# JJKK1313/DiTreeOnlinePlanner

Measured on AMD Instinct MI355X. Metric: candidate tree-expansions/sec (carmaze, H=32), higher is better.
Workload: dtype f16x3; 1 GPU; cfgs/carmaze.yaml + fm_policy flow sampler (K=1), batch=1024 candidates per GPU, H=32 (4 chunks x 8 steps), boxes.csv 20x20, 1024-node tree snapshot, seeded random weights; batch_per_gpu=1024, global_batch=1024, edge_length=32, action_horizon=8, pred_horizon=64, flow_steps=1, tree_nodes=1024, parallelism=candidates sharded x1

## Files before the change

### ditreeonlineplanner_amd/csrc/denoise.h

```cpp
#pragma once
#include <hip/hip_runtime.h>
#include <stdint.h>

enum { MODE_BIAS = 0, MODE_GN_MISH = 1, MODE_GN_MISH_FILM = 2, MODE_GN_MISH_RES = 3 };

enum { ST_BF16 = 0, ST_F32 = 1, ST_F16 = 2 };
static inline int fmt_make(int st, bool split) { return st | (split ? 4 : 0); }
static inline __host__ __device__ int fmt_st(int f) { return f & 3; }
static inline __host__ __device__ bool fmt_split(int f) { return (f & 4) != 0; }
static inline int fmt_es(int f) { return fmt_st(f) == ST_F32 ? 4 : 2; }

struct ConvGemmParams {
  const void* A;
  int lda;
  int in_Lp;
  int in_stride;
  int in_off;
  int taps, Cin;
  const void* W;
  void* Out;
  int ldc;
  int out_Lp, out_stride, out_off;
  int out_coff;
  int L;
  int M, N;
  const float* bias;
  int mode;
  const float* gamma;
  const float* beta;
  int group_ch;
  float eps;
  const float* film;
  int film_ld, film_off;
  const void* Res;
  int ldres, res_Lp, res_off;
  int out_f32;
  int dbg;
  int c2d, c2_H, c2_W, c2_OW, c2_OHW, c2_stride, c2_pad;
  signed char c2_kh[12], c2_kw[12];
  const void* zero;
  long long a_plane, w_plane, out_plane, res_plane;
  float w_scale;
  int splitk;
  long long slab_stride;
  float* sk_ws;
  int* sk_cnt;
  int* sat;
};

void denoise_set_dry_run(bool on);
void launch_conv_gemm(const ConvGemmParams& p, int fmt, hipStream_t s);
bool conv2d_small_eligible(int fmt);
int conv_gemm_kind(const ConvGemmParams& p, int fmt);
bool conv_gemm_supported(const ConvGemmParams& p, int fmt);
void launch_prep_sample(const float* x, void* A0, int B, int P, int D, int fmt, long long plane, hipStream_t s, int* sat = nullptr);
void launch_time_embed(float t, const float* W1, const float* b1, const float* W2, const float* b2, float* out,
                       hipStream_t s);
void launch_prep_cond(const float* temb, const float* map_emb, int E, int E_ld, const float* cond, int G, void* out, int B,
                      int Kpad, int fmt, long long plane, hipStream_t s, int* sat = nullptr);
struct FlowStep {
  int mode;
  float dt;
  float sb, sa, c0, c1, sigma;
  const float* z;
  long long z_row;
  const int* z_idx;
  int z_row0;
};
void launch_final_proj_flow(const void* Y, int C, int Lp, long long plane, const float* W, const float* bias, int D, float* x,
                            FlowStep fs, const double* act_norm , double* actions, int B, int P, int fmt,
                            hipStream_t s);
struct TapList {
  int n;
  signed char kh[49], kw[49];
};
void launch_gn1d(void* x, int ld, int Lp, int row_off, int coff, int L, int C, const float* gamma, const float* beta, float eps,
                 int mode, const float* film, int film_ld, int film_off, const void* res, int ldres, int res_Lp, int res_off,
                 int B, int fmt, long long x_plane, long long res_plane, hipStream_t s, int* sat = nullptr);
void launch_encoder_stem(const float* lm, int n, const float* W, const float* gamma, const float* beta, void* out, int B, float eps,
                         int fmt, long long plane, hipStream_t s, int* sat = nullptr);
void launch_im2col2d(const void* in, bool src_f32, void* out, int B, int H, int W, int C, const TapList& taps, int stride,
                     int pad, int OH, int OW, int Kpad, int fmt, hipStream_t s);
// ... 9 lines not shown
```

### ditreeonlineplanner_amd/csrc/denoise_host.hip

```cpp
#include <algorithm>
#include <cmath>
#include <cstring>
#include <functional>
#include <map>
#include <sstream>
#include <thread>

#include "denoise.h"
#include "ditree_internal.h"

namespace {

struct HostParam {
  std::vector<int64_t> dims;
  const float* data = nullptr;
  int64_t n = 0;
};

struct Act {
  void* p = nullptr;
  int L = 0, C = 0;
  int ld = 0, coff = 0;
  bool padded = true;
  long long plane = 0;
// ... 41 lines not shown
  int bgran = 16;
  int ufmt = 0, efmt = 0;
  std::vector<void*> allocs;
  std::map<std::string, Act> named;
  std::map<std::string, Packed> dev_w;
  std::map<std::string, float*> dev_f;
  std::vector<std::function<void(int, int, hipStream_t)>> unet_ops;
  std::vector<std::function<void(int, int, int, hipStream_t)>> enc_ops;
  static constexpr int ENC_SUBS = 4;
  int sub_cap = 0;
  size_t col_region = 0, gout_region = 0;
  hipStream_t aux[ENC_SUBS] = {nullptr, nullptr, nullptr, nullptr};
  hipEvent_t ev_fork = nullptr, ev_join[ENC_SUBS] = {nullptr, nullptr, nullptr, nullptr};
  std::function<void(int, int, hipStream_t)> film_op;
  float* x_cur = nullptr;
  float* temb = nullptr;
  float temb_t = -1.0f;
  float* map_emb = nullptr;
  int E_ld = 400;
  float* film = nullptr;
  void* condA = nullptr;
  long long cond_plane = 0;
  int condK = 0, film_cols = 0;
  Act final_h;
  const float* lm_ptr = nullptr;
  void* zero_row = nullptr;
  static constexpr int SAT_SLOTS = 256;
  int* sat_flags = nullptr;
  int *sat_cond = nullptr, *sat_sample = nullptr;
  std::vector<std::string> sat_names;
  int* sat_slot(const std::string& layer, int fmt) {
    if (fmt_st(fmt) != ST_F16 || sat_flags == nullptr) return nullptr;
    for (size_t i = 0; i < sat_names.size(); ++i)
      if (sat_names[i] == layer) return sat_flags + i;
    if ((int)sat_names.size() >= SAT_SLOTS) return sat_flags + SAT_SLOTS - 1;
    sat_names.push_back(layer);
    return sat_flags + sat_names.size() - 1;
  }
  int last_splitk[4] = {1, 1, 1, 1};
  long long last_slab[4] = {0, 0, 0, 0};
  bool prof_on = false;
  int prof_mode = 0;
  std::vector<hipEvent_t> prof_ev;
  size_t prof_used = 0;
  double prof_ms_done[3] = {0, 0, 0};
  int64_t prof_launches_done[3] = {0, 0, 0};
// ... 98 lines not shown
    if (it == params.end()) throw std::runtime_error("missing parameter " + name);
    return it->second;
  }
  bool has(const std::string& name) const { return params.count(name) != 0; }

  void* dalloc(size_t bytes, bool zero = true) {
    void* p = nullptr;
    if (hipMalloc(&p, bytes ? bytes : 16) != hipSuccess) throw std::runtime_error("hipMalloc failed");
    if (zero && hipMemset(p, 0, bytes ? bytes : 16) != hipSuccess) throw std::runtime_error("hipMemset failed");
    allocs.push_back(p);
    return p;
  }
  void free_workspace() {
    for (void* p : allocs) hipFree(p);
    allocs.clear();
    sk_ws = nullptr;
    sk_cnt = nullptr;
    named.clear();
    dev_w.clear();
    dev_f.clear();
    enc_ops.clear();
    unet_ops.clear();
    film_op = nullptr;
    sat_flags = sat_cond = sat_sample = nullptr;
    sat_names.clear();
    prec = -1;
    Bmax = 0;
    Buser = 0;
    temb_t = -1.0f;
  }

  float* upload_f32(const std::string& key, const float* src, int64_t n) {
    auto it = dev_f.find(key);
    if (it != dev_f.end()) return it->second;
    float* d = (float*)dalloc((size_t)n * 4, false);
    if (hipMemcpy(d, src, (size_t)n * 4, hipMemcpyHostToDevice) != hipSuccess) throw std::runtime_error("memcpy");
    dev_f[key] = d;
    return d;
  }
  float* vec(const std::string& name) {
    const HostParam& hp = P_(name);
    return upload_f32(name, hp.data, hp.n);
  }

  template <class F>
  Packed pack(const std::string& key, int fmt, int N, int T, int Cin_pad, F get) {
// ... 218 lines not shown
    default: throw std::runtime_error("unknown precision");
  }
  sat_flags = (int*)dalloc(SAT_SLOTS * sizeof(int));
  sat_cond = sat_slot("cond_encoder input: Mish(time | map embedding | observation)", ufmt);
  sat_sample = sat_slot("sample (the noisy action sequence)", ufmt);
  const int C0 = dims[0], C1 = dims[1], C2 = dims[2];
  const int L0 = P, L1 = P / 2, L2 = P / 4;
  if (P % 16 != 0 || P < 16 || P > 256 || (256 % P) != 0) throw std::runtime_error("pred_horizon must be 16, 32, 64, 128 or 256");
  bgran = fmt_st(ufmt) != ST_F32 ? std::max(16, 1024 / P) : 16;
  Buser = Bmax_;
  Bmax = (Bmax_ + bgran - 1) / bgran * bgran;
  {
    const long long per_sample = std::max({(long long)(L2 + 2) * 2 * C2, (long long)(L1 + 2) * 2 * C1, (long long)(L0 + 2) * C0,
                                           (long long)L0 * 64}) * fmt_es(ufmt);
    long long cap = std::min<long long>(8192, 0x7f000000LL / per_sample);
    cap = cap / 256 * 256;
    if (cap < 256) throw std::runtime_error("denoiser too large for one 256-sample work unit");
    if (Bmax > cap) Bmax = (int)cap;
  }
  if (fmt_split(ufmt) && ((C0 | C1 | C2) & 255) != 0)
    throw std::runtime_error("the split precisions need down_dims that are multiples of 256 (halo / gemm16 tiles)");
  x_cur = (float*)dalloc((size_t)Bmax * P * D * 4);
  temb = (float*)dalloc(256 * 4);
  condK = (cond_dim + 63) / 64 * 64;
  const int Brows = (Bmax + 255) / 256 * 256;
  E_ld = fmt_split(efmt) ? (E + 255) / 256 * 256 : E;
  map_emb = (float*)dalloc((size_t)Brows * E_ld * 4);
  cond_plane = planes() == 2 ? (long long)Brows * condK * es() : 0;
  condA = dalloc((size_t)Brows * condK * es() * planes());

  std::vector<std::string> crbs = {"unet.down_modules.0.0", "unet.down_modules.0.1", "unet.down_modules.1.0",
                                   "unet.down_modules.1.1", "unet.down_modules.2.0", "unet.down_modules.2.1",
                                   "unet.mid_modules.0",    "unet.mid_modules.1",    "unet.up_modules.0.0",
                                   "unet.up_modules.0.1",   "unet.up_modules.1.0",   "unet.up_modules.1.1"};
  film_cols = 0;
  std::vector<int> film_offs;
  for (auto& c : crbs) {
    film_offs.push_back(film_cols);
    film_cols += (int)P_(c + ".cond_encoder.1.weight").dims[0];
  }
  film = (float*)dalloc((size_t)Brows * film_cols * 4);
  {
    std::vector<const float*> wsrc, bsrc;
    std::vector<int> rows;
    for (auto& c : crbs) {
      wsrc.push_back(P_(c + ".cond_encoder.1.weight").data);
      bsrc.push_back(P_(c + ".cond_encoder.1.bias").data);
      rows.push_back((int)P_(c + ".cond_encoder.1.weight").dims[0]);
    }
    std::vector<int> start(rows.size());
    for (size_t i = 0, a = 0; i < rows.size(); ++i) { start[i] = (int)a; a += rows[i]; }
    const int cd = cond_dim;
    const Packed wp = pack("film.all", ufmt, film_cols, 1, condK, [=](int n, int, int ci) {
      size_t i = std::upper_bound(start.begin(), start.end(), n) - start.begin() - 1;
      return ci < cd ? wsrc[i][(size_t)(n - start[i]) * cd + ci] : 0.0f;
    });
    std::vector<float> ball(film_cols);
    for (size_t i = 0; i < rows.size(); ++i) std::memcpy(ball.data() + start[i], bsrc[i], (size_t)rows[i] * 4);
    float* bd = upload_f32("film.bias", ball.data(), film_cols);
    ConvGemmParams p{};
    p.A = condA; p.lda = condK; p.in_Lp = 0; p.in_stride = 1; p.in_off = 0; p.taps = 1; p.Cin = condK;
    set_w(p, wp); p.a_plane = cond_plane;
    p.Out = film; p.ldc = film_cols; p.out_Lp = 0; p.out_stride = 1; p.out_off = 0;
    p.N = film_cols; p.bias = bd; p.mode = MODE_BIAS; p.out_f32 = 1;
    const int uf = ufmt;
    film_op = [this, p, uf](int, int Bp, hipStream_t s) mutable {
      const int Mr = fmt_st(uf) == ST_F32 ? Bp : (Bp + 255) / 256 * 256;
      p.M = Mr; p.L = Mr; p.in_Lp = Mr; p.out_Lp = Mr;
      run_gemm(p, uf, s);
    };
  }

  int fc = 0;
  Act a0;
  a0.L = L0; a0.C = 64; a0.ld = 64; a0.coff = 0; a0.padded = false; a0.fmt = ufmt;
  a0.plane = planes() == 2 ? (long long)Bmax * L0 * 64 * es() : 0;
  a0.p = dalloc((size_t)Bmax * L0 * 64 * es() * planes());
  named["a0"] = a0;
  {
    const std::string pre = "unet.down_modules.0.0";
    const HostParam& w = P_(pre + ".blocks.0.block.0.weight");
    const float* wd = w.data;
// ... 142 lines not shown
        float* goutr = gout + (size_t)reg * goutreg;
        ConvGemmParams p{};
        const int M = Bn * OH * OH;
        if (implicit) {
          p.A = (const char*)in + (size_t)b0 * H * H * Cin * E_; p.lda = Cin; p.taps = tl.n; p.Cin = Cin; p.a_plane = in_plane;
          p.c2d = 1; p.c2_H = H; p.c2_W = H; p.c2_OW = OH; p.c2_OHW = OH * OH; p.c2_stride = stride; p.c2_pad = pad;
          for (int t = 0; t < tl.n; ++t) { p.c2_kh[t] = tl.kh[t]; p.c2_kw[t] = tl.kw[t]; }
          p.zero = zr;
          const int nk_total = tl.n * (Cin / 64);
          const int tiles = ((1024 * OH * OH + 255) / 256) * ((Cout + 255) / 256);
          static int sk_target = -1, sk_cap = 8;
          if (sk_target < 0) {
            const char* e = getenv("DITREE_SPLITK_TARGET");
            sk_target = (e && atoi(e) > 0) ? atoi(e) : 256;
            const char* c = getenv("DITREE_SPLITK_CAP");
            if (c && atoi(c) > 0) sk_cap = atoi(c);
          }
          int sk = std::max(1, std::min(std::min(sk_cap, nk_total / 2), std::max(1, sk_target / tiles)));
          while (sk > 1 && (size_t)sk * OH * OH * Cout > gout_per_sample) --sk;
          if (sk > 1) {
            const int per = (nk_total + sk - 1) / sk;
            sk = (nk_total + per - 1) / per;
          }
          static int use_split = -1;
          if (use_split < 0) { const char* e = getenv("DITREE_SPLITK"); use_split = (e && !atoi(e)) ? 0 : 1; }
          if (conv2d_small_eligible(pr)) {
            static int small_target = -1;
            if (small_target < 0) { const char* e = getenv("DITREE_C2D_TARGET"); small_target = (e && atoi(e) > 0) ? atoi(e) : 768; }
            const int tiles64 = ((1024 * OH * OH + 63) / 64) * (Cout / 64);
            sk = std::max(1, std::min(std::min(8, nk_total / 2), small_target / tiles64));
            while (sk > 1 && (size_t)sk * OH * OH * Cout > gout_per_sample) --sk;
            if (sk > 1) {
              const int per = (nk_total + sk - 1) / sk;
              sk = (nk_total + per - 1) / per;
            }
          }
          if (!use_split) sk = 1;
          p.splitk = sk;
          p.slab_stride = (long long)M * Cout;
          last_splitk[reg] = sk;
          last_slab[reg] = p.slab_stride;
        } else {
          last_splitk[reg] = 1;
          last_slab[reg] = 0;
        }
        if (!implicit) {
          note_other();
          if (in == nullptr)
            launch_im2col2d(*lm_slot + (size_t)b0 * H * H, true, colr, Bn, H, H, 1, tl, stride, pad, OH, OH, Kpad, pr, s);
          else
            launch_im2col2d((const char*)in + (size_t)b0 * H * H * Cin * E_, false, colr, Bn, H, H, Cin, tl, stride, pad,
// ... 296 lines not shown
        HIP_TRY(ctx, hipEventCreateWithFlags(&st->ev_join[i], hipEventDisableTiming));
      }
      HIP_TRY(ctx, hipEventCreateWithFlags(&st->ev_fork, hipEventDisableTiming));
    }
    if (nsub > 1) HIP_TRY(ctx, hipEventRecord(st->ev_fork, s));
    for (int i = 0; i < nsub; ++i) {
      const int b0 = i * per, bn = std::min(per, B - b0);
      if (bn <= 0) break;
      hipStream_t si = (i == 0) ? s : st->aux[i];
      if (i > 0) HIP_TRY(ctx, hipStreamWaitEvent(si, st->ev_fork, 0));
      for (auto& op : st->enc_ops) op(b0, bn, i, si);
      if (i > 0) {
        HIP_TRY(ctx, hipEventRecord(st->ev_join[i], si));
        HIP_TRY(ctx, hipStreamWaitEvent(s, st->ev_join[i], 0));
      }
    }
  }
  for (int k = 0; k < K; ++k) {
    const float t = t0[k] * t_scale;
    if (t != st->temb_t) {
      launch_time_embed(t, st->dev_f["unet.diffusion_step_encoder.1.weight"], st->dev_f["unet.diffusion_step_encoder.1.bias"],
                        st->dev_f["unet.diffusion_step_encoder.3.weight"], st->dev_f["unet.diffusion_step_encoder.3.bias"],
                        st->temb, s);
      st->temb_t = K == 1 ? t : -1.0f;
    }
    st->note_other();
    launch_prep_cond(st->temb, st->map_emb, st->E, st->E_ld, cond, st->G, st->condA, B, st->condK, uf, st->cond_plane, s,
                     st->sat_cond);
    st->film_op(B, Bp, s);
    st->note_other();
    launch_prep_sample(st->x_cur, st->named["a0"].p, Bp, st->P, st->D, uf, st->named["a0"].plane, s,
                       st->sat_sample);
    for (auto& op : st->unet_ops) op(B, Bp, s);
    const bool last = (k == K - 1);
    st->note_other();
    FlowStep fs{};
    fs.mode = raw ? 1 : 0;
    fs.dt = dt[k];
    if (st->ddpm_coef) {
      const float* c = st->ddpm_coef + 5 * k;
      fs.mode = 2; fs.sb = c[0]; fs.sa = c[1]; fs.c0 = c[2]; fs.c1 = c[3]; fs.sigma = c[4];
      fs.z = st->ddpm_z ? st->ddpm_z + (long long)k * st->ddpm_z_step : nullptr;
      fs.z_row = st->ddpm_z_row; fs.z_idx = noise_idx; fs.z_row0 = st->ddpm_row0;
      if (fs.sigma != 0.0f && !fs.z) return set_err(ctx, DITREE_E_ARG, "denoise: a DDPM step with sigma > 0 needs step noise");
    }
    launch_final_proj_flow(st->final_h.p, st->final_h.C, st->final_h.Lp(), st->final_h.plane, st->dev_f["unet.final_conv.1.weight"],
                           st->dev_f["unet.final_conv.1.bias"], st->D, st->x_cur, fs, act_norm,
                           (last && actions) ? actions : nullptr, B, st->P, uf, s);
  }
  } catch (const std::exception& e) {
// ... 199 lines not shown
```

### ditreeonlineplanner_amd/csrc/denoise_kernels.hip

```cpp
#include <cstdlib>
#include <type_traits>

#include <stdexcept>

#include "denoise.h"

static thread_local bool g_dn_dry_run = false;
void denoise_set_dry_run(bool on) { g_dn_dry_run = on; }
#define DN_LAUNCH(...) do { if (!g_dn_dry_run) hipLaunchKernelGGL(__VA_ARGS__); } while (0)

typedef __attribute__((ext_vector_type(8))) __bf16 bf16x8_t;
typedef __attribute__((ext_vector_type(8))) _Float16 half8_t;
typedef __attribute__((ext_vector_type(8))) short short8_t;
typedef __attribute__((ext_vector_type(4))) short short4_t;
typedef __attribute__((ext_vector_type(16))) float f32x16_t;
typedef __attribute__((ext_vector_type(4))) float f32x4_t;
typedef __attribute__((ext_vector_type(2))) float f32x2_t;
typedef __attribute__((ext_vector_type(2))) _Float16 half2_t;
typedef __attribute__((ext_vector_type(2))) short short2_t;

#define GLOBAL_AS __attribute__((address_space(1)))
#define LDS_AS __attribute__((address_space(3)))

__device__ __forceinline__ unsigned short f2bf(float f) {
// ... 1325 lines not shown
#pragma unroll
      for (int mb = 0; mb < 4; ++mb)
#pragma unroll
        for (int j = 0; j < 8; ++j) acc[mb][j] += *(const f32x4_t*)(sl + ((mb * 8 + j) * 512 + tid) * 4);
    }
    if (tid == 0) p.sk_cnt[tile] = 0;
  }
  gemm_epilogue16<ET, true, SHORT>(p, acc, smem, tm, tn, tid, lane, r4, h4, wm, wn);
#ifdef HALO16_STAMP
  __syncthreads();
  if (tid == 0) {
    const unsigned long long xs3 = __builtin_amdgcn_s_memrealtime();
    const unsigned int k = atomicAdd(&g_x3_count, 1u);
    if (k < X3_STAMP_MAX) {
      g_x3_stamp[k][0] = xs0; g_x3_stamp[k][1] = xs1; g_x3_stamp[k][2] = xs2; g_x3_stamp[k][3] = xs3;
      g_x3_stamp[k][4] = ((unsigned long long)nv << 32) | blockIdx.x;
      g_x3_stamp[k][5] = ((unsigned long long)__builtin_amdgcn_s_getreg((31 << 11) | 20) << 32) |
                         (unsigned int)__builtin_amdgcn_s_getreg((31 << 11) | 4);
    }
  }
#endif
}

template <int ET, bool SPLIT>
__global__ void __launch_bounds__(256) conv2d_small_kernel(ConvGemmParams p) {
  extern __shared__ __attribute__((aligned(16))) char smem[];
  constexpr int STAGE = 16384;
  constexpr int CK = SPLIT ? 32 : 64;
  const int tid = threadIdx.x, lane = tid & 63;
  const int w = __builtin_amdgcn_readfirstlane(tid >> 6);
  const int r5 = lane & 31, h = lane >> 5;
  const int wm = w >> 1, wn = w & 1;
  const int ntn = p.N >> 6;
  const int tm = blockIdx.x / ntn, tn = blockIdx.x - tm * ntn;
  const int kpt = p.Cin / CK;
  const long long K = (long long)p.taps * p.Cin;
  int k0 = 0, nk = p.taps * kpt;
  long long out_extra = 0;
  if (p.splitk > 1) {
    const int per = (nk + p.splitk - 1) / p.splitk;
    k0 = blockIdx.y * per;
    nk = min(nk - k0, per);
    out_extra = (long long)blockIdx.y * p.slab_stride;
  }

  const char* a_base[2];
  int ih0[2], iw0[2];
  const char* w_src[2];
  int slot_b[2];
  long long plane_a[2];
#pragma unroll
  for (int q = 0; q < 2; ++q) {
    const int r = (2 * w + q) * 8 + (lane >> 3);
    const int slot = (lane & 7) ^ ((r >> 1) & 7);
    slot_b[q] = SPLIT ? (slot & 3) * 16 : slot * 16;
    plane_a[q] = (SPLIT && (slot & 4)) ? p.a_plane : 0;
    const long long plane_w = (SPLIT && (slot & 4)) ? p.w_plane : 0;
    int m = tm * 64 + r;
    m = m < p.M ? m : p.M - 1;
    const int b = m / p.c2_OHW, rem = m - b * p.c2_OHW;
    const int oh = rem / p.c2_OW, ow = rem - oh * p.c2_OW;
    a_base[q] = (const char*)p.A + (long long)b * p.c2_H * p.c2_W * p.Cin * 2;
    ih0[q] = oh * p.c2_stride - p.c2_pad;
    iw0[q] = ow * p.c2_stride - p.c2_pad;
    w_src[q] = (const char*)p.W + ((long long)(tn * 64 + r) * K) * 2 + slot_b[q] + plane_w;
  }
  auto issue = [&](int kl) {
    const int k = k0 + kl;
    const int tap = k / kpt, kin = k - tap * kpt;
    const int kh = p.c2_kh[tap], kw = p.c2_kw[tap];
    char* st = smem + (kl % 3) * STAGE;
#pragma unroll
    for (int q = 0; q < 2; ++q) {
      const int ih = ih0[q] + kh, iw = iw0[q] + kw;
      const bool ok = ih >= 0 && ih < p.c2_H && iw >= 0 && iw < p.c2_W;
      const char* src = ok ? a_base[q] + ((long long)(ih * p.c2_W + iw) * p.Cin + kin * CK) * 2 + plane_a[q] : (const char*)p.zero;
      __builtin_amdgcn_global_load_lds((const GLOBAL_AS void*)(src + slot_b[q]), (LDS_AS void*)(st + (2 * w + q) * 1024), 16, 0, 0);
    }
#pragma unroll
    for (int q = 0; q < 2; ++q)
      __builtin_amdgcn_global_load_lds((const GLOBAL_AS void*)(w_src[q] + (long long)k * (CK * 2)),
                                       (LDS_AS void*)(st + 8192 + (2 * w + q) * 1024), 16, 0, 0);
  };

  f32x16_t acc;
#pragma unroll
  for (int i = 0; i < 16; ++i) acc[i] = 0.0f;
  const int a_row = wm * 32 + r5, b_row = wn * 32 + r5;
  const int a_off = a_row * 128, b_off = 8192 + b_row * 128;
  const int sa = (a_row >> 1) & 7, sb = (b_row >> 1) & 7;

  issue(0);
  if (nk > 1) issue(1);
  for (int k = 0; k < nk; ++k) {
    if (k + 1 < nk) asm volatile("s_waitcnt vmcnt(4)" ::: "memory");
    else asm volatile("s_waitcnt vmcnt(0)" ::: "memory");
    __builtin_amdgcn_s_barrier();
    if (k + 2 < nk) issue(k + 2);
    const char* st = smem + (k % 3) * STAGE;
    if constexpr (SPLIT) {
      short8_t af[4], bf[4];
#pragma unroll
      for (int ks = 0; ks < 4; ++ks) {
        af[ks] = *(const short8_t*)(st + a_off + ((((ks << 1) | h) ^ sa) << 4));
        bf[ks] = *(const short8_t*)(st + b_off + ((((ks << 1) | h) ^ sb) << 4));
      }
#pragma unroll
      for (int kk = 0; kk < 2; ++kk) acc = mfma32<ET>(af[kk], bf[kk + 2], acc);
#pragma unroll
      for (int kk = 0; kk < 2; ++kk) acc = mfma32<ET>(af[kk], bf[kk], acc);
#pragma unroll
      for (int kk = 0; kk < 2; ++kk) acc = mfma32<ET>(af[kk + 2], bf[kk], acc);
    } else {
#pragma unroll
      for (int ks = 0; ks < 4; ++ks) {
        const short8_t af = *(const short8_t*)(st + a_off + ((((ks << 1) | h) ^ sa) << 4));
        const short8_t bf = *(const short8_t*)(st + b_off + ((((ks << 1) | h) ^ sb) << 4));
        acc = mfma32<ET>(af, bf, acc);
      }
    }
    asm volatile("s_waitcnt lgkmcnt(0)" ::: "memory");
  }

  const int n = tn * 64 + wn * 32 + r5;
  float bias = (p.bias != nullptr && k0 == 0) ? p.bias[n] : 0.0f;
#pragma unroll
  for (int i = 0; i < 16; ++i) {
    const int m = tm * 64 + wm * 32 + (i & 3) + 8 * (i >> 2) + 4 * h;
    if (m < p.M) ((float*)p.Out)[out_extra + (long long)m * p.ldc + p.out_coff + n] = (ET == 1 ? acc[i] * p.w_scale : acc[i]) + bias;
  }
}

template <int ET, bool SPLIT, bool SHORT = false>
__global__ void __launch_bounds__(512, 2) gemm16_kernel(ConvGemmParams p) {
  extern __shared__ __attribute__((aligned(16))) char smem[];
  constexpr int BUF = 32768, W_BASE = 2 * BUF;
  const int tid = threadIdx.x, lane = tid & 63;
  const int w = __builtin_amdgcn_readfirstlane(tid >> 6);
  const int r4 = lane & 15, h4 = lane >> 4;
  const int wm = w >> 1, wn = w & 1;
  const int ntn = p.N >> 8, ntm = p.M >> 8;
  const int tile = xcd_remap_strips(blockIdx.x, ntm, ntn, p.dbg);
  const int tm = tile / ntn, tn = tile - tm * ntn;
  constexpr int KB = SPLIT ? 64 : 128;
  const int nc = SPLIT ? (p.Cin >> 5) : (p.Cin >> 6), nk = p.taps * nc;
  const unsigned a_plane = (unsigned)p.a_plane, w_plane = (unsigned)p.w_plane;
  const long long K = (long long)p.taps * p.Cin;

  long long a_tile0;
  {
    const int m0 = tm * 256;
    const int b0 = m0 / p.L, l0 = m0 - b0 * p.L;
// ... 205 lines not shown
  if (nk >= 2) step(Tt{}, Ff{}, nk - 2);
  step(Ff{}, Ff{}, nk - 1);
  __syncthreads();
  gemm_epilogue16<ET, SPLIT, SHORT>(p, acc, smem, tm, tn, tid, lane, r4, h4, wm, wn);
}
static bool gemm16_eligible(const ConvGemmParams& p, int fmt) {
  const bool short_ok = p.L == 8 || p.L == 4;
  return fmt_st(fmt) != ST_F32 && !p.c2d && (!p.out_f32 || p.mode == MODE_BIAS) && p.taps >= 1 && p.taps <= 3 && (p.M & 255) == 0 &&
         (p.N & 255) == 0 && (p.Cin & 63) == 0 && ((p.L & 15) == 0 || short_ok) && p.M > 0 &&
         (p.mode == MODE_BIAS || (256 % p.L) == 0);
}
static bool halo_eligible(const ConvGemmParams& p, int fmt) {
  static const bool l8_off = [] { const char* e = getenv("DITREE_HALO_L8"); return e && atoi(e) == 0; }();
  static const bool l4_off = [] { const char* e = getenv("DITREE_HALO_L4"); return e && atoi(e) == 0; }();
  const bool l_ok = p.L >= 16 || (p.L == 8 && fmt_split(fmt) && !l8_off) || (p.L == 4 && fmt_split(fmt) && !l4_off && p.splitk <= 1);
  return fmt_st(fmt) != ST_F32 && !p.c2d && p.taps == 3 && p.in_stride == 1 && p.in_Lp == p.L + 2 && (256 % p.L) == 0 &&
         l_ok && (p.M & 255) == 0 && (p.N & 255) == 0 && (p.Cin & 63) == 0 && p.Cin >= 192;
}
bool conv2d_small_eligible(int fmt) { return fmt_st(fmt) != ST_F32; }
int conv_gemm_kind(const ConvGemmParams& p, int fmt) { return halo_eligible(p, fmt) ? 0 : (p.c2d ? 2 : 1); }
bool conv_gemm_supported(const ConvGemmParams& p, int fmt) {
  return !fmt_split(fmt) || halo_eligible(p, fmt) || gemm16_eligible(p, fmt) ||
         (p.c2d && (p.N & 63) == 0 && (p.Cin & 63) == 0 && p.out_f32 && p.mode == MODE_BIAS);
}

static void ensure_lds_attrs() {
  static bool done[64] = {};
  int dev = 0;
  hipGetDevice(&dev);
  if (dev < 0 || dev >= 64 || done[dev]) return;
  done[dev] = true;
  const hipFuncAttribute at = hipFuncAttributeMaxDynamicSharedMemorySize;
  hipFuncSetAttribute((const void*)conv_gemm_kernel<0, false>, at, 131072);
  hipFuncSetAttribute((const void*)conv_gemm_kernel<1, false>, at, 131072);
  hipFuncSetAttribute((const void*)conv_gemm_kernel<2, false>, at, 131072);
  hipFuncSetAttribute((const void*)conv_gemm_kernel<0, true>, at, 131072);
  hipFuncSetAttribute((const void*)conv_gemm_kernel<1, true>, at, 131072);
  hipFuncSetAttribute((const void*)conv_gemm_kernel<2, true>, at, 131072);
  hipFuncSetAttribute((const void*)conv3_halo16_kernel<0, false>, at, 147456);
  hipFuncSetAttribute((const void*)conv3_halo16_kernel<1, false>, at, 147456);
  hipFuncSetAttribute((const void*)conv3_halo16x3_kernel<0>, at, 147456);
  hipFuncSetAttribute((const void*)conv3_halo16x3_kernel<1>, at, 147456);
  hipFuncSetAttribute((const void*)conv3_halo16x3_kernel<0, true>, at, 147456);
  hipFuncSetAttribute((const void*)conv3_halo16x3_kernel<1, true>, at, 147456);
  hipFuncSetAttribute((const void*)conv3_halo16x3_kernel<0, false, true>, at, 147456);
  hipFuncSetAttribute((const void*)conv3_halo16x3_kernel<1, false, true>, at, 147456);
// ... 49 lines not shown
  if (gemm16_eligible(p, fmt) && (p.L & 15) != 0) {
    if (split) {
      if (f16) DN_LAUNCH((gemm16_kernel<1, true, true>), grid, block, 131072, s, p);
      else DN_LAUNCH((gemm16_kernel<0, true, true>), grid, block, 131072, s, p);
    } else {
      if (f16) DN_LAUNCH((gemm16_kernel<1, false, true>), grid, block, 131072, s, p);
      else DN_LAUNCH((gemm16_kernel<0, false, true>), grid, block, 131072, s, p);
    }
    return;
  }
  if (gemm16_eligible(p, fmt)) {
    if (split) {
      if (f16) DN_LAUNCH((gemm16_kernel<1, true>), grid, block, 131072, s, p);
      else DN_LAUNCH((gemm16_kernel<0, true>), grid, block, 131072, s, p);
    } else {
      if (f16) DN_LAUNCH((gemm16_kernel<1, false>), grid, block, 131072, s, p);
      else DN_LAUNCH((gemm16_kernel<0, false>), grid, block, 131072, s, p);
    }
    return;
  }
  if (p.mode >= MODE_GN_MISH && (p.L & 15) != 0)
    throw std::runtime_error("conv_gemm: a fused GroupNorm epilogue at L = 8 / 4 exists on the gemm16 tile only (whole 256-row tiles)");
  if (p.c2d && conv2d_small_eligible(fmt) && (p.N & 63) == 0 && (p.Cin & 63) == 0 && p.out_f32 && p.mode == MODE_BIAS) {
    const dim3 g2(((p.M + 63) >> 6) * (p.N >> 6), p.splitk > 1 ? p.splitk : 1);
    if (split) {
      if (f16) DN_LAUNCH((conv2d_small_kernel<1, true>), g2, dim3(256), 3 * 16384, s, p);
      else DN_LAUNCH((conv2d_small_kernel<0, true>), g2, dim3(256), 3 * 16384, s, p);
    } else {
      if (f16) DN_LAUNCH((conv2d_small_kernel<1, false>), g2, dim3(256), 3 * 16384, s, p);
      else DN_LAUNCH((conv2d_small_kernel<0, false>), g2, dim3(256), 3 * 16384, s, p);
    }
    return;
  }
  if (split) throw std::runtime_error("conv_gemm: a split GEMM of this shape fits no tile (conv_gemm_supported is the contract)");
  if (p.c2d) {
    const dim3 grid2(ntm * ntn, p.splitk > 1 ? p.splitk : 1);
    if (st == ST_F32) DN_LAUNCH((conv_gemm_kernel<1, true>), grid2, block, 131072, s, p);
    else if (f16) DN_LAUNCH((conv_gemm_kernel<2, true>), grid2, block, 131072, s, p);
    else DN_LAUNCH((conv_gemm_kernel<0, true>), grid2, block, 131072, s, p);
    return;
  }
  if (st == ST_F32) DN_LAUNCH((conv_gemm_kernel<1, false>), grid, block, 131072, s, p);
  else if (f16) DN_LAUNCH((conv_gemm_kernel<2, false>), grid, block, 131072, s, p);
  else DN_LAUNCH((conv_gemm_kernel<0, false>), grid, block, 131072, s, p);
}

template <int FMT>
__device__ __forceinline__ void store_elem(void* base, long long idx, float v, long long plane = 0) {
  constexpr int ST = FMT & 3;
  if constexpr (ST == ST_F32) {
    ((float*)base)[idx] = v;
  } else {
    constexpr int ET = ST == ST_F16 ? 1 : 0;
// ... 341 lines not shown
    emb[tid] = (tid < 128) ? sinf(a) : cosf(a);
  }
  __syncthreads();
  {
    float s = b1[tid];
    const float* wr = W1 + (long long)tid * 256;
    for (int k = 0; k < 256; ++k) s += wr[k] * emb[k];
    hid[tid] = mish_f<1>(s);
  }
  __syncthreads();
  if (tid < 256) {
    float s = b2[tid];
    const float* wr = W2 + (long long)tid * 1024;
    for (int k = 0; k < 1024; ++k) s += wr[k] * hid[k];
    out[tid] = s;
  }
}
void launch_time_embed(float t, const float* W1, const float* b1, const float* W2, const float* b2, float* out,
                       hipStream_t s) {
  DN_LAUNCH(time_embed_kernel, dim3(1), dim3(1024), 0, s, t, W1, b1, W2, b2, out);
}

template <int PREC>
__global__ void prep_cond_kernel(const float* __restrict__ temb, const float* __restrict__ map_emb, int E, int E_ld,
                                 const float* __restrict__ cond, int G, void* __restrict__ out, int B, int Kpad, long long plane,
                                 int* __restrict__ sat) {
  const int b = blockIdx.x;
  float satm = 0.0f;
  for (int k = threadIdx.x; k < Kpad; k += blockDim.x) {
    float v = 0.f;
    bool live = true;
    if (k < 256) v = temb[k];
    else if (k < 256 + E) v = map_emb[(long long)b * E_ld + (k - 256)];
    else if (k < 256 + E + G) v = cond[(long long)b * G + (k - 256 - E)];
    else live = false;
    store_elem<PREC>(out, (long long)b * Kpad + k, live ? MISH_OF(PREC)(v) : 0.f, plane, satm);
  }
  if constexpr ((PREC & 3) == ST_F16) sat_flush(sat, satm);
}
void launch_prep_cond(const float* temb, const float* map_emb, int E, int E_ld, const float* cond, int G, void* out, int B,
                      int Kpad, int fmt, long long plane, hipStream_t s, int* sat) {
#define CALL(F) DN_LAUNCH(prep_cond_kernel<F>, dim3(B), dim3(256), 0, s, temb, map_emb, E, E_ld, cond, G, out, B, Kpad, plane, sat)
  DISPATCH_FMT(fmt, CALL)
#undef CALL
}

struct ActNormArg { double mu[8], sg[8]; };
template <int PREC, int D>
__global__ void __launch_bounds__(256) final_proj_flow_kernel(const void* __restrict__ Y, int C, int Lp, long long plane,
                                                              const float* __restrict__ W ,
                                                              const float* __restrict__ bias,
                                                              float* __restrict__ x , FlowStep fs,
                                                              ActNormArg nm, double* __restrict__ actions, int B, int P) {
  const long long pos = blockIdx.x * 4LL + (threadIdx.x >> 6);
  const int lane = threadIdx.x & 63;
  if (pos >= (long long)B * P) return;
  const int b = (int)(pos / P), l = (int)(pos - (long long)b * P);
  const long long row = (long long)b * Lp + l + 1;
  float s[D];
#pragma unroll
  for (int d = 0; d < D; ++d) s[d] = 0.f;
  for (int c = lane * 8; c < C; c += 512) {
    float y[8];
    if constexpr ((PREC & 3) == ST_F32) {
      const f32x4_t y0 = *(const f32x4_t*)((const float*)Y + row * C + c), y1 = *(const f32x4_t*)((const float*)Y + row * C + c + 4);
#pragma unroll
      for (int j = 0; j < 4; ++j) { y[j] = y0[j]; y[4 + j] = y1[j]; }
// ... 269 lines not shown
```

Before: 19410 candidate expansions/s.

## Fold FiLM time-embedding into bias, skip dead conv2d taps, deepen staging ring

The timestep embedding is the same for every candidate, so its contribution to the FiLM GEMM is precomputed once per step into a bias vector. This removes 256 K-columns from the per-candidate cond GEMM. The small implicit Conv2d kernel now orders tiles by output position so each block can skip taps that fall in padding instead of loading zeros. It also gains a configurable 3-5 stage cp.async-style LDS ring, and a few env lookups move into workspace setup. The trade-off is extra template instantiations, a small extra kernel per timestep, and a larger LDS footprint when more stages are chosen.

```diff
diff --git a/ditreeonlineplanner_amd/csrc/denoise.h b/ditreeonlineplanner_amd/csrc/denoise.h
--- a/ditreeonlineplanner_amd/csrc/denoise.h
+++ b/ditreeonlineplanner_amd/csrc/denoise.h
@@ -37,6 +37,7 @@
   int out_f32;
   int dbg;
   int c2d, c2_H, c2_W, c2_OW, c2_OHW, c2_stride, c2_pad;
+  int c2_B, c2_stages;
   signed char c2_kh[12], c2_kw[12];
   const void* zero;
   long long a_plane, w_plane, out_plane, res_plane;
@@ -56,8 +57,9 @@
 void launch_prep_sample(const float* x, void* A0, int B, int P, int D, int fmt, long long plane, hipStream_t s, int* sat = nullptr);
 void launch_time_embed(float t, const float* W1, const float* b1, const float* W2, const float* b2, float* out,
                        hipStream_t s);
-void launch_prep_cond(const float* temb, const float* map_emb, int E, int E_ld, const float* cond, int G, void* out, int B,
+void launch_prep_cond(const float* temb, int T, const float* map_emb, int E, int E_ld, const float* cond, int G, void* out, int B,
                       int Kpad, int fmt, long long plane, hipStream_t s, int* sat = nullptr);
+void launch_film_tbias(const float* temb, const float* Wt, const float* bias, float* out, int N, hipStream_t s);
 struct FlowStep {
   int mode;
   float dt;
diff --git a/ditreeonlineplanner_amd/csrc/denoise_host.hip b/ditreeonlineplanner_amd/csrc/denoise_host.hip
--- a/ditreeonlineplanner_amd/csrc/denoise_host.hip
+++ b/ditreeonlineplanner_amd/csrc/denoise_host.hip
@@ -87,6 +87,12 @@
   void* condA = nullptr;
   long long cond_plane = 0;
   int condK = 0, film_cols = 0;
+  bool film_fold = true, c2d_deadtaps = true, enc_splitk = true;
+  int c2d_stages = 3, c2d_target = 768;
+  int film_T = 256;
+  float* film_tbias = nullptr;
+  const float* film_wt = nullptr;
+  const float* film_bias0 = nullptr;
   Act final_h;
   const float* lm_ptr = nullptr;
   void* zero_row = nullptr;
@@ -231,6 +237,8 @@
     enc_ops.clear();
     unet_ops.clear();
     film_op = nullptr;
+    film_tbias = nullptr;
+    film_wt = film_bias0 = nullptr;
     sat_flags = sat_cond = sat_sample = nullptr;
     sat_names.clear();
     prec = -1;
@@ -495,7 +503,18 @@
     throw std::runtime_error("the split precisions need down_dims that are multiples of 256 (halo / gemm16 tiles)");
   x_cur = (float*)dalloc((size_t)Bmax * P * D * 4);
   temb = (float*)dalloc(256 * 4);
-  condK = (cond_dim + 63) / 64 * 64;
+  {
+    auto env_int = [](const char* name, int dflt) { const char* e = getenv(name); return e ? atoi(e) : dflt; };
+    film_fold = env_int("DITREE_FILM_FOLD", 1) != 0;
+    c2d_deadtaps = env_int("DITREE_C2D_DEADTAPS", 1) != 0;
+    c2d_stages = env_int("DITREE_C2D_STAGES", 3);
+    if (c2d_stages < 3 || c2d_stages > 5) throw std::runtime_error("DITREE_C2D_STAGES must be 3, 4 or 5");
+    c2d_target = env_int("DITREE_C2D_TARGET", 768);
+    if (c2d_target <= 0) c2d_target = 768;
+    enc_splitk = env_int("DITREE_SPLITK", 1) != 0;
+  }
+  film_T = film_fold ? 0 : 256;
+  condK = (cond_dim - 256 + film_T + 63) / 64 * 64;
   const int Brows = (Bmax + 255) / 256 * 256;
   E_ld = fmt_split(efmt) ? (E + 255) / 256 * 256 : E;
   map_emb = (float*)dalloc((size_t)Brows * E_ld * 4);
@@ -523,14 +542,23 @@
     }
     std::vector<int> start(rows.size());
     for (size_t i = 0, a = 0; i < rows.size(); ++i) { start[i] = (int)a; a += rows[i]; }
-    const int cd = cond_dim;
+    const int cd = cond_dim, toff = 256 - film_T;
     const Packed wp = pack("film.all", ufmt, film_cols, 1, condK, [=](int n, int, int ci) {
       size_t i = std::upper_bound(start.begin(), start.end(), n) - start.begin() - 1;
-      return ci < cd ? wsrc[i][(size_t)(n - start[i]) * cd + ci] : 0.0f;
+      return ci + toff < cd ? wsrc[i][(size_t)(n - start[i]) * cd + ci + toff] : 0.0f;
     });
     std::vector<float> ball(film_cols);
     for (size_t i = 0; i < rows.size(); ++i) std::memcpy(ball.data() + start[i], bsrc[i], (size_t)rows[i] * 4);
     float* bd = upload_f32("film.bias", ball.data(), film_cols);
+    if (film_fold) {
+      std::vector<float> wt((size_t)film_cols * 256);
+      for (size_t i = 0; i < rows.size(); ++i)
+        for (int r = 0; r < rows[i]; ++r) std::memcpy(wt.data() + (size_t)(start[i] + r) * 256, wsrc[i] + (size_t)r * cd, 256 * 4);
+      film_wt = upload_f32("film.wt", wt.data(), (int64_t)film_cols * 256);
+      film_bias0 = bd;
+      film_tbias = (float*)dalloc((size_t)film_cols * 4);
+      bd = film_tbias;
+    }
     ConvGemmParams p{};
     p.A = condA; p.lda = condK; p.in_Lp = 0; p.in_stride = 1; p.in_off = 0; p.taps = 1; p.Cin = condK;
     set_w(p, wp); p.a_plane = cond_plane;
@@ -719,11 +747,11 @@
             const int per = (nk_total + sk - 1) / sk;
             sk = (nk_total + per - 1) / per;
           }
-          static int use_split = -1;
-          if (use_split < 0) { const char* e = getenv("DITREE_SPLITK"); use_split = (e && !atoi(e)) ? 0 : 1; }
+          const int use_split = enc_splitk ? 1 : 0;
           if (conv2d_small_eligible(pr)) {
-            static int small_target = -1;
-            if (small_target < 0) { const char* e = getenv("DITREE_C2D_TARGET"); small_target = (e && atoi(e) > 0) ? atoi(e) : 768; }
+            const int small_target = c2d_target;
+            p.c2_B = c2d_deadtaps ? Bn : 0;
+            p.c2_stages = c2d_stages;
             const int tiles64 = ((1024 * OH * OH + 63) / 64) * (Cout / 64);
             sk = std::max(1, std::min(std::min(8, nk_total / 2), small_target / tiles64));
             while (sk > 1 && (size_t)sk * OH * OH * Cout > gout_per_sample) --sk;
@@ -1066,10 +1094,11 @@
       launch_time_embed(t, st->dev_f["unet.diffusion_step_encoder.1.weight"], st->dev_f["unet.diffusion_step_encoder.1.bias"],
                         st->dev_f["unet.diffusion_step_encoder.3.weight"], st->dev_f["unet.diffusion_step_encoder.3.bias"],
                         st->temb, s);
+      if (st->film_fold) launch_film_tbias(st->temb, st->film_wt, st->film_bias0, st->film_tbias, st->film_cols, s);
       st->temb_t = K == 1 ? t : -1.0f;
     }
     st->note_other();
-    launch_prep_cond(st->temb, st->map_emb, st->E, st->E_ld, cond, st->G, st->condA, B, st->condK, uf, st->cond_plane, s,
+    launch_prep_cond(st->temb, st->film_T, st->map_emb, st->E, st->E_ld, cond, st->G, st->condA, B, st->condK, uf, st->cond_plane, s,
                      st->sat_cond);
     st->film_op(B, Bp, s);
     st->note_other();
diff --git a/ditreeonlineplanner_amd/csrc/denoise_kernels.hip b/ditreeonlineplanner_amd/csrc/denoise_kernels.hip
--- a/ditreeonlineplanner_amd/csrc/denoise_kernels.hip
+++ b/ditreeonlineplanner_amd/csrc/denoise_kernels.hip
@@ -1371,7 +1371,15 @@
 #endif
 }
 
-template <int ET, bool SPLIT>
+template <int NST>
+__device__ __forceinline__ void c2d_wait_stage(int ahead) {
+  static_assert(NST >= 3 && NST <= 5, "ring depth");
+  if (NST >= 5 && ahead >= 3) asm volatile("s_waitcnt vmcnt(12)" ::: "memory");
+  else if (NST >= 4 && ahead >= 2) asm volatile("s_waitcnt vmcnt(8)" ::: "memory");
+  else if (ahead >= 1) asm volatile("s_waitcnt vmcnt(4)" ::: "memory");
+  else asm volatile("s_waitcnt vmcnt(0)" ::: "memory");
+}
+template <int ET, bool SPLIT, int NST, bool PM>
 __global__ void __launch_bounds__(256) conv2d_small_kernel(ConvGemmParams p) {
   extern __shared__ __attribute__((aligned(16))) char smem[];
   constexpr int STAGE = 16384;
@@ -1382,6 +1390,15 @@
   const int wm = w >> 1, wn = w & 1;
   const int ntn = p.N >> 6;
   const int tm = blockIdx.x / ntn, tn = blockIdx.x - tm * ntn;
+  int pos = 0, bt = 0, ihu = 0, iwu = 0;
+  if constexpr (PM) {
+    const int nbt = (p.c2_B + 63) >> 6;
+    pos = tm / nbt;
+    bt = tm - pos * nbt;
+    const int oh = pos / p.c2_OW, ow = pos - oh * p.c2_OW;
+    ihu = oh * p.c2_stride - p.c2_pad;
+    iwu = ow * p.c2_stride - p.c2_pad;
+  }
   const int kpt = p.Cin / CK;
   const long long K = (long long)p.taps * p.Cin;
   int k0 = 0, nk = p.taps * kpt;
@@ -1392,6 +1409,27 @@
     nk = min(nk - k0, per);
     out_extra = (long long)blockIdx.y * p.slab_stride;
   }
+  unsigned long long khp = 0, kwp = 0;
+#pragma unroll
+  for (int t = 0; t < 12; ++t) {
+    khp |= (unsigned long long)(p.c2_kh[t] & 15) << (4 * t);
+    kwp |= (unsigned long long)(p.c2_kw[t] & 15) << (4 * t);
+  }
+  auto tap_kh = [&](int t) { return (int)((khp >> (4 * t)) & 15); };
+  auto tap_kw = [&](int t) { return (int)((kwp >> (4 * t)) & 15); };
+  unsigned live = ~0u;
+  int nlive = nk;
+  if constexpr (PM) {
+    live = 0u;
+    nlive = 0;
+    for (int t = 0; t < p.taps; ++t) {
+      const int ih = ihu + tap_kh(t), iw = iwu + tap_kw(t);
+      if (ih >= 0 && ih < p.c2_H && iw >= 0 && iw < p.c2_W) {
+        live |= 1u << t;
+        nlive += max(0, min(k0 + nk, (t + 1) * kpt) - max(k0, t * kpt));
+      }
+    }
+  }
 
   const char* a_base[2];
   int ih0[2], iw0[2];
@@ -1405,31 +1443,58 @@
     slot_b[q] = SPLIT ? (slot & 3) * 16 : slot * 16;
     plane_a[q] = (SPLIT && (slot & 4)) ? p.a_plane : 0;
     const long long plane_w = (SPLIT && (slot & 4)) ? p.w_plane : 0;
-    int m = tm * 64 + r;
-    m = m < p.M ? m : p.M - 1;
-    const int b = m / p.c2_OHW, rem = m - b * p.c2_OHW;
-    const int oh = rem / p.c2_OW, ow = rem - oh * p.c2_OW;
+    int b;
+    if constexpr (PM) {
+      b = min(bt * 64 + r, p.c2_B - 1);
+      ih0[q] = ihu;
+      iw0[q] = iwu;
+    } else {
+      int m = tm * 64 + r;
+      m = m < p.M ? m : p.M - 1;
+      b = m / p.c2_OHW;
+      const int rem = m - b * p.c2_OHW;
+      const int oh = rem / p.c2_OW, ow = rem - oh * p.c2_OW;
+      ih0[q] = oh * p.c2_stride - p.c2_pad;
+      iw0[q] = ow * p.c2_stride - p.c2_pad;
+    }
     a_base[q] = (const char*)p.A + (long long)b * p.c2_H * p.c2_W * p.Cin * 2;
-    ih0[q] = oh * p.c2_stride - p.c2_pad;
-    iw0[q] = ow * p.c2_stride - p.c2_pad;
+    if constexpr (PM) a_base[q] += plane_a[q] + slot_b[q];
     w_src[q] = (const char*)p.W + ((long long)(tn * 64 + r) * K) * 2 + slot_b[q] + plane_w;
   }
-  auto issue = [&](int kl) {
-    const int k = k0 + kl;
-    const int tap = k / kpt, kin = k - tap * kpt;
-    const int kh = p.c2_kh[tap], kw = p.c2_kw[tap];
-    char* st = smem + (kl % 3) * STAGE;
-#pragma unroll
-    for (int q = 0; q < 2; ++q) {
-      const int ih = ih0[q] + kh, iw = iw0[q] + kw;
-      const bool ok = ih >= 0 && ih < p.c2_H && iw >= 0 && iw < p.c2_W;
-      const char* src = ok ? a_base[q] + ((long long)(ih * p.c2_W + iw) * p.Cin + kin * CK) * 2 + plane_a[q] : (const char*)p.zero;
-      __builtin_amdgcn_global_load_lds((const GLOBAL_AS void*)(src + slot_b[q]), (LDS_AS void*)(st + (2 * w + q) * 1024), 16, 0, 0);
+  int c_tap = k0 / kpt, c_kin = k0 - c_tap * kpt, c_slot = 0;
+  if constexpr (PM) {
+    if (!((live >> c_tap) & 1u)) {
+      c_kin = 0;
+      do ++c_tap; while (c_tap < p.taps && !((live >> c_tap) & 1u));
+    }
+  }
+  auto issue = [&]() {
+    const int k = c_tap * kpt + c_kin;
+    const int kh = tap_kh(c_tap), kw = tap_kw(c_tap);
+    char* st = smem + c_slot * STAGE;
+    if constexpr (PM) {
+      const long long src_off = ((long long)((ihu + kh) * p.c2_W + (iwu + kw)) * p.Cin + c_kin * CK) * 2;
+#pragma unroll
+      for (int q = 0; q < 2; ++q)
+        __builtin_amdgcn_global_load_lds((const GLOBAL_AS void*)(a_base[q] + src_off), (LDS_AS void*)(st + (2 * w + q) * 1024), 16, 0, 0);
+    } else {
+#pragma unroll
+      for (int q = 0; q < 2; ++q) {
+        const int ih = ih0[q] + kh, iw = iw0[q] + kw;
+        const bool ok = ih >= 0 && ih < p.c2_H && iw >= 0 && iw < p.c2_W;
+        const char* src = ok ? a_base[q] + ((long long)(ih * p.c2_W + iw) * p.Cin + c_kin * CK) * 2 + plane_a[q] : (const char*)p.zero;
+        __builtin_amdgcn_global_load_lds((const GLOBAL_AS void*)(src + slot_b[q]), (LDS_AS void*)(st + (2 * w + q) * 1024), 16, 0, 0);
+      }
     }
 #pragma unroll
     for (int q = 0; q < 2; ++q)
       __builtin_amdgcn_global_load_lds((const GLOBAL_AS void*)(w_src[q] + (long long)k * (CK * 2)),
                                        (LDS_AS void*)(st + 8192 + (2 * w + q) * 1024), 16, 0, 0);
+    c_slot = c_slot + 1 == NST ? 0 : c_slot + 1;
+    if (++c_kin == kpt) {
+      c_kin = 0;
+      do ++c_tap; while (PM && c_tap < p.taps && !((live >> c_tap) & 1u));
+    }
   };
 
   f32x16_t acc;
@@ -1439,14 +1504,16 @@
   const int a_off = a_row * 128, b_off = 8192 + b_row * 128;
   const int sa = (a_row >> 1) & 7, sb = (b_row >> 1) & 7;
 
-  issue(0);
-  if (nk > 1) issue(1);
-  for (int k = 0; k < nk; ++k) {
-    if (k + 1 < nk) asm volatile("s_waitcnt vmcnt(4)" ::: "memory");
-    else asm volatile("s_waitcnt vmcnt(0)" ::: "memory");
+#pragma unroll
+  for (int i = 0; i < NST - 1; ++i)
+    if (i < nlive) issue();
+  int r_slot = 0;
+  for (int k = 0; k < nlive; ++k) {
+    c2d_wait_stage<NST>(min(NST - 2, nlive - 1 - k));
     __builtin_amdgcn_s_barrier();
-    if (k + 2 < nk) issue(k + 2);
-    const char* st = smem + (k % 3) * STAGE;
+    if (k + NST - 1 < nlive) issue();
+    const char* st = smem + r_slot * STAGE;
+    r_slot = r_slot + 1 == NST ? 0 : r_slot + 1;
     if constexpr (SPLIT) {
       short8_t af[4], bf[4];
 #pragma unroll
@@ -1475,8 +1542,18 @@
   float bias = (p.bias != nullptr && k0 == 0) ? p.bias[n] : 0.0f;
 #pragma unroll
   for (int i = 0; i < 16; ++i) {
-    const int m = tm * 64 + wm * 32 + (i & 3) + 8 * (i >> 2) + 4 * h;
-    if (m < p.M) ((float*)p.Out)[out_extra + (long long)m * p.ldc + p.out_coff + n] = (ET == 1 ? acc[i] * p.w_scale : acc[i]) + bias;
+    const int rr = wm * 32 + (i & 3) + 8 * (i >> 2) + 4 * h;
+    bool ok;
+    long long m;
+    if constexpr (PM) {
+      const int b = bt * 64 + rr;
+      ok = b < p.c2_B;
+      m = (long long)b * p.c2_OHW + pos;
+    } else {
+      m = tm * 64 + rr;
+      ok = m < p.M;
+    }
+    if (ok) ((float*)p.Out)[out_extra + m * p.ldc + p.out_coff + n] = (ET == 1 ? acc[i] * p.w_scale : acc[i]) + bias;
   }
 }
 
@@ -1728,6 +1805,32 @@
 bool conv_gemm_supported(const ConvGemmParams& p, int fmt) {
   return !fmt_split(fmt) || halo_eligible(p, fmt) || gemm16_eligible(p, fmt) ||
          (p.c2d && (p.N & 63) == 0 && (p.Cin & 63) == 0 && p.out_f32 && p.mode == MODE_BIAS);
+}
+
+template <int ET, bool SP, int NST>
+static void launch_c2d_small_n(const ConvGemmParams& p, dim3 g2, hipStream_t s) {
+  if (NST * 16384 > 65536) {
+    static bool done[64] = {};
+    int dev = 0;
+    hipGetDevice(&dev);
+    if (dev >= 0 && dev < 64 && !done[dev]) {
+      done[dev] = true;
+      hipFuncSetAttribute((const void*)conv2d_small_kernel<ET, SP, NST, true>, hipFuncAttributeMaxDynamicSharedMemorySize, NST * 16384);
+      hipFuncSetAttribute((const void*)conv2d_small_kernel<ET, SP, NST, false>, hipFuncAttributeMaxDynamicSharedMemorySize, NST * 16384);
+    }
+  }
+  if (p.c2_B > 0) DN_LAUNCH((conv2d_small_kernel<ET, SP, NST, true>), g2, dim3(256), NST * 16384, s, p);
+  else DN_LAUNCH((conv2d_small_kernel<ET, SP, NST, false>), g2, dim3(256), NST * 16384, s, p);
+}
+template <int ET, bool SP>
+static void launch_c2d_small(const ConvGemmParams& p, dim3 g2, hipStream_t s) {
+  switch (p.c2_stages) {
+    case 0:
+    case 3: launch_c2d_small_n<ET, SP, 3>(p, g2, s); break;
+    case 4: launch_c2d_small_n<ET, SP, 4>(p, g2, s); break;
+    case 5: launch_c2d_small_n<ET, SP, 5>(p, g2, s); break;
+    default: throw std::runtime_error("conv_gemm: the implicit Conv2d staging ring has 3, 4 or 5 stages");
+  }
 }
 
 static void ensure_lds_attrs() {
@@ -1823,13 +1926,15 @@
   if (p.mode >= MODE_GN_MISH && (p.L & 15) != 0)
     throw std::runtime_error("conv_gemm: a fused GroupNorm epilogue at L = 8 / 4 exists on the gemm16 tile only (whole 256-row tiles)");
   if (p.c2d && conv2d_small_eligible(fmt) && (p.N & 63) == 0 && (p.Cin & 63) == 0 && p.out_f32 && p.mode == MODE_BIAS) {
-    const dim3 g2(((p.M + 63) >> 6) * (p.N >> 6), p.splitk > 1 ? p.splitk : 1);
+    if (p.c2_B > 0 && p.M != p.c2_B * p.c2_OHW) throw std::runtime_error("conv_gemm: implicit Conv2d rows do not match its sample count");
+    const int ntm64 = p.c2_B > 0 ? p.c2_OHW * ((p.c2_B + 63) >> 6) : (p.M + 63) >> 6;
+    const dim3 g2(ntm64 * (p.N >> 6), p.splitk > 1 ? p.splitk : 1);
     if (split) {
-      if (f16) DN_LAUNCH((conv2d_small_kernel<1, true>), g2, dim3(256), 3 * 16384, s, p);
-      else DN_LAUNCH((conv2d_small_kernel<0, true>), g2, dim3(256), 3 * 16384, s, p);
+      if (f16) launch_c2d_small<1, true>(p, g2, s);
+      else launch_c2d_small<0, true>(p, g2, s);
     } else {
-      if (f16) DN_LAUNCH((conv2d_small_kernel<1, false>), g2, dim3(256), 3 * 16384, s, p);
-      else DN_LAUNCH((conv2d_small_kernel<0, false>), g2, dim3(256), 3 * 16384, s, p);
+      if (f16) launch_c2d_small<1, false>(p, g2, s);
+      else launch_c2d_small<0, false>(p, g2, s);
     }
     return;
   }
@@ -2217,7 +2322,7 @@
 }
 
 template <int PREC>
-__global__ void prep_cond_kernel(const float* __restrict__ temb, const float* __restrict__ map_emb, int E, int E_ld,
+__global__ void prep_cond_kernel(const float* __restrict__ temb, int T, const float* __restrict__ map_emb, int E, int E_ld,
                                  const float* __restrict__ cond, int G, void* __restrict__ out, int B, int Kpad, long long plane,
                                  int* __restrict__ sat) {
   const int b = blockIdx.x;
@@ -2225,19 +2330,35 @@
   for (int k = threadIdx.x; k < Kpad; k += blockDim.x) {
     float v = 0.f;
     bool live = true;
-    if (k < 256) v = temb[k];
-    else if (k < 256 + E) v = map_emb[(long long)b * E_ld + (k - 256)];
-    else if (k < 256 + E + G) v = cond[(long long)b * G + (k - 256 - E)];
+    if (k < T) v = temb[k];
+    else if (k < T + E) v = map_emb[(long long)b * E_ld + (k - T)];
+    else if (k < T + E + G) v = cond[(long long)b * G + (k - T - E)];
     else live = false;
     store_elem<PREC>(out, (long long)b * Kpad + k, live ? MISH_OF(PREC)(v) : 0.f, plane, satm);
   }
   if constexpr ((PREC & 3) == ST_F16) sat_flush(sat, satm);
 }
-void launch_prep_cond(const float* temb, const float* map_emb, int E, int E_ld, const float* cond, int G, void* out, int B,
+void launch_prep_cond(const float* temb, int T, const float* map_emb, int E, int E_ld, const float* cond, int G, void* out, int B,
                       int Kpad, int fmt, long long plane, hipStream_t s, int* sat) {
-#define CALL(F) DN_LAUNCH(prep_cond_kernel<F>, dim3(B), dim3(256), 0, s, temb, map_emb, E, E_ld, cond, G, out, B, Kpad, plane, sat)
+#define CALL(F) DN_LAUNCH(prep_cond_kernel<F>, dim3(B), dim3(256), 0, s, temb, T, map_emb, E, E_ld, cond, G, out, B, Kpad, plane, sat)
   DISPATCH_FMT(fmt, CALL)
 #undef CALL
+}
+
+__global__ void __launch_bounds__(256) film_tbias_kernel(const float* __restrict__ temb, const float* __restrict__ Wt,
+                                                         const float* __restrict__ bias, float* __restrict__ out, int N) {
+  const int n = blockIdx.x * 4 + (threadIdx.x >> 6), lane = threadIdx.x & 63;
+  if (n >= N) return;
+  const float* wr = Wt + (long long)n * 256;
+  float s = 0.0f;
+#pragma unroll
+  for (int j = 0; j < 4; ++j) s = fmaf(wr[lane + 64 * j], mish_f<1>(temb[lane + 64 * j]), s);
+#pragma unroll
+  for (int o = 32; o >= 1; o >>= 1) s += __shfl_xor(s, o);
+  if (lane == 0) out[n] = bias[n] + s;
+}
+void launch_film_tbias(const float* temb, const float* Wt, const float* bias, float* out, int N, hipStream_t s) {
+  DN_LAUNCH(film_tbias_kernel, dim3((N + 3) / 4), dim3(256), 0, s, temb, Wt, bias, out, N);
 }
 
 struct ActNormArg { double mu[8], sg[8]; };
```

Result: no change. 19590 candidate expansions/s (median of 6 runs) (+1.0%).
